# wujian16/Cornell-MOE

Measured on AMD Instinct MI355X. Metric: q-KG gradient evals/s (n=1000,d=8,q=4,10k MC), higher is better.
Workload: dtype f64

## Files before the change

### cornell_moe_amd/csrc/kg.hip

```cpp
#include "kg.hpp"

#include <algorithm>
#include <array>
#include <atomic>
#include <exception>
#include <mutex>
#include <thread>
#include <memory>
#include <optional>
#include <chrono>
#include <cmath>
#include <cstdlib>

#include "device_cov.hpp"
#include "fastmath.hpp"
#include "gemm128.hpp"
#include "kg_mc.hpp"
#include "kg_state.hpp"

namespace moe {

static thread_local int t_ens_members_hint = 1;
int ensemble_members_hint() { return t_ens_members_hint; }
void set_ensemble_members_hint(int members) { t_ens_members_hint = members > 1 ? members : 1; }
// ... 394 lines not shown
struct kg_dir_kernel_body {
  static __device__ __forceinline__ void run(const VIdx blockIdx, const VIdx gridDim, const void*, const KgTailParams& P, double* __restrict__ part, int slices) {
    __shared__ double red[4];
    const int k = blockIdx.x, e = blockIdx.y, sl = blockIdx.z;
    const int per = (P.num_local + slices - 1) / slices;
    const int i_lo = sl * per, i_hi = min(P.num_local, i_lo + per);
    const int m = P.m, g1 = 1 + P.g, d = P.cp.dim;
    const double* Xu = P.blob + (long)e * P.rec.stride + P.rec.XuP + (long)k * DP;
    DerivList none;
    none.g = 0;
    double xk[DP];
  #pragma unroll
    for (int kk = 0; kk < DP; ++kk) xk[kk] = Xu[kk];
    for (int b = 0; b < g1; ++b) {
      double acc[DP];
  #pragma unroll
      for (int dd = 0; dd < DP; ++dd) acc[dd] = 0.0;
      for (int i = i_lo + threadIdx.x; i < i_hi; i += 256) {
        const long w = (long)e * P.num_local + i;
        const double* xs = P.best_point + w * DP;
        double diff[DP];
        double r2 = 0.0;
  #pragma unroll
        for (int kk = 0; kk < DP; ++kk) {
          diff[kk] = xk[kk] - xs[kk];
          r2 = fma(diff[kk] * diff[kk], P.cp.inv_l2[kk], r2);
        }
        const Radial rd = radial_scalars(P.cp.type, P.cp.alpha, r2);
        const double bt = P.beta[w * m + k * g1 + b];
  #pragma unroll
        for (int dd = 0; dd < DP; ++dd)
          if (dd < d) acc[dd] = fma(bt, grad_cov_entry<DP>(P.cp, rd, diff, b, 0, dd, P.derivs, none), acc[dd]);
      }
  #pragma unroll
      for (int dd = 0; dd < DP; ++dd) {
        if (dd < d) {
          const double tot = block_sum_256(acc[dd], red);
          if (threadIdx.x == 0) part[((long)e * P.ngrad + (k * g1 + b) * d + dd) * slices + sl] = tot;
        }
      }
    }
  }
};
template <int DP>
__global__ __launch_bounds__(256) void kg_dir_kernel(KgTailParams P, double* __restrict__ part, int slices) {
  kg_dir_kernel_body<DP>::run(MOE_VBLOCK, MOE_VGRID, nullptr, P, part, slices);
}

inline int dir_slices(int num_local) { return std::max(1, std::min(kDirSlices, (num_local + 255) / 256)); }
inline double* dir_partials(const KgTailParams& P) {
  return P.TBpart + (long)P.E * (P.chunks + 1) * (long)P.m * P.N;
}

template <int DP>
void launch_dir(const KgTailParams& P, hipStream_t s) {
  const int slices = dir_slices(P.num_local);
  launch_kernel_ens<kg_dir_kernel_body<DP>, 256>(kg_dir_kernel<DP>, dim3(P.q, P.E, slices), dim3(256), 0, s, P, dir_partials(P), slices);
}

template <int DP, int MU>
void launch_sw_inst(const KgTailParams& P, hipStream_t s) {
  dim3 grid((P.num_local + P.sw_chunk - 1) / P.sw_chunk, P.E);
  const size_t shm = (P.SW == nullptr) ? sizeof(double) * (size_t)P.N * P.m : 0;
  auto kern = kg_sw_kernel<DP, MU>;
  if (shm > 48 * 1024)
    MOE_HIP_CHECK(hipFuncSetAttribute(reinterpret_cast<const void*>(kern), hipFuncAttributeMaxDynamicSharedMemorySize, (int)shm));
  launch_kernel_ens<kg_sw_kernel_body<DP, MU>, 256>(kern, grid, dim3(256), shm, s, P);
}

template <int DP>
void launch_sw_dp(const KgTailParams& P, hipStream_t s) {
  if (P.m <= 4)
    launch_sw_inst<DP, 4>(P, s);
  else if (P.m <= 8)
    launch_sw_inst<DP, 8>(P, s);
  else if (P.m <= 16)
    launch_sw_inst<DP, 16>(P, s);
  else if (P.m <= 32)
    launch_sw_inst<DP, 32>(P, s);
  else if (P.m <= 64)
    launch_sw_inst<DP, 64>(P, s);
  else {
    if (P.SW == nullptr) throw Error(MOE_ERR_RUNTIME, "m > 64 needs the precomputed W^T T");
    dim3 grid((P.num_local + P.sw_chunk - 1) / P.sw_chunk, P.E);
    launch_kernel_ens<kg_sw_kernel_body<DP, 1, 2>, 256>(kg_sw_kernel<DP, 1, 2>, grid, dim3(256), 0, s, P);
  }
  launch_dir<DP>(P, s);
}

void launch_tail(const KgTailParams& P, hipStream_t s) {
  switch (P.cp.dp) {
    case 4: launch_sw_dp<4>(P, s); break;
    case 8: launch_sw_dp<8>(P, s); break;
    case 12: launch_sw_dp<12>(P, s); break;
    case 16: launch_sw_dp<16>(P, s); break;
    case 24: launch_sw_dp<24>(P, s); break;
    case 32: launch_sw_dp<32>(P, s); break;
    default: throw Error(MOE_ERR_RUNTIME, "unsupported padded dimension");
  }
  dim3 gtb((P.N + 255) / 256, P.chunks, P.E);
  if (P.m <= 4)
    launch_kernel_ens<kg_tb_kernel_body<4>, 256>(kg_tb_kernel<4>, gtb, dim3(256), 0, s, P, 0);
  else if (P.m <= 8)
    launch_kernel_ens<kg_tb_kernel_body<8>, 256>(kg_tb_kernel<8>, gtb, dim3(256), 0, s, P, 0);
  else if (P.m <= 16)
    launch_kernel_ens<kg_tb_kernel_body<16>, 256>(kg_tb_kernel<16>, gtb, dim3(256), 0, s, P, 0);
// ... 73 lines not shown
__global__ __launch_bounds__(256) void kg_fused_sample_kernel(KgTailParams P, const double* __restrict__ X, int n,
                                                             double* __restrict__ SWpart) {
  kg_fused_sample_kernel_body<DP, MU, COV>::run(MOE_VBLOCK, MOE_VGRID, nullptr, P, X, n, SWpart);
}

template <int DP, int MU, int COV>
struct kg_fused_c_kernel_body {
  static __device__ __forceinline__ void run(const VIdx blockIdx, const VIdx gridDim, const void*, const KgTailParams& P, const double* __restrict__ SWpart, int slices) {
    __shared__ double etab[kExpTabLen];
    const int e = blockIdx.y, m = P.m;
    const int i = blockIdx.x * 256 + threadIdx.x;
    if (threadIdx.x < kExpTabLen) etab[threadIdx.x] = kExp2Tab64[threadIdx.x];
    __syncthreads();
    if (i >= P.num_local) return;
    const long w = (long)e * P.num_local + i;
    double xs[DP], sw[MU], cv[MU];
  #pragma unroll
    for (int k = 0; k < DP; ++k) xs[k] = P.best_point[w * DP + k] * P.cp.inv_l[k];
  #pragma unroll
    for (int c = 0; c < MU; ++c) {
      sw[c] = 0.0;
      for (int sl = 0; sl < slices; ++sl) sw[c] += SWpart[(w * slices + sl) * MU + c];
    }
    const double* rec = P.blob + (long)e * P.rec.stride;
    const double* Lsm = rec + P.rec.L;
  #pragma unroll
    for (int r = 0; r < MU; ++r) {
      cv[r] = 0.0;
      if (r < m) {
        const double* Xu = rec + P.rec.XuP + (long)r * DP;
        double r2 = 1.0e-300;
  #pragma unroll
        for (int k = 0; k < DP; ++k) {
          const double dlt = Xu[k] * P.cp.inv_l[k] - xs[k];
          r2 = fma(dlt, dlt, r2);
        }
        double R = P.cp.alpha * (radial_base<COV>(r2, etab) - sw[r]);
  #pragma unroll
        for (int c = 0; c < MU; ++c)
          if (c < r) R -= Lsm[r + c * m] * cv[c];
        cv[r] = R / Lsm[r + r * m];
        P.C[w * m + r] = cv[r];
      }
    }
  }
};
template <int DP, int MU, int COV>
__global__ __launch_bounds__(256) void kg_fused_c_kernel(KgTailParams P, const double* __restrict__ SWpart, int slices) {
  kg_fused_c_kernel_body<DP, MU, COV>::run(MOE_VBLOCK, MOE_VGRID, nullptr, P, SWpart, slices);
}

template <int DP, int MU, int COV>
struct kg_fused_point_kernel_body {
  static __device__ __forceinline__ void run(const VIdx blockIdx, const VIdx gridDim, const void*, const KgTailParams& P, const double* __restrict__ X, int n) {
    __shared__ double etab[kExpTabLen];
    __shared__ double St[kFusedTile][DP];
    __shared__ double Bt[kFusedTile][MU];
    const int row = blockIdx.x * 256 + threadIdx.x;
    const int chunk = blockIdx.y, e = blockIdx.z;
    const int m = P.m;
    const int i0 = chunk * P.chunk_len, cnt = min(P.num_local - i0, P.chunk_len);
    if (threadIdx.x < kExpTabLen) etab[threadIdx.x] = kExp2Tab64[threadIdx.x];
    for (int t = threadIdx.x; t < kFusedTile * DP; t += 256) {
      const int ii = t / DP, k = t % DP;
      St[ii][k] = (ii < cnt) ? P.best_point[((long)e * P.num_local + i0 + ii) * DP + k] * P.cp.inv_l[k] : 0.0;
    }
    for (int t = threadIdx.x; t < kFusedTile * MU; t += 256) {
      const int ii = t / MU, c = t % MU;
      Bt[ii][c] = (ii < cnt && c < m) ? P.beta[((long)e * P.num_local + i0 + ii) * m + c] : 0.0;
    }
    __syncthreads();
    const bool ok = row < n;
    double xr[DP], acc[MU];
  #pragma unroll
    for (int k = 0; k < DP; ++k) xr[k] = ok ? X[(long)row * DP + k] * P.cp.inv_l[k] : 0.0;
  #pragma unroll
    for (int c = 0; c < MU; ++c) acc[c] = 0.0;
  #pragma unroll 2
    for (int ii = 0; ii < cnt; ++ii) {
      double r2 = 1.0e-300;
  #pragma unroll
      for (int k = 0; k < DP; ++k) {
        const double dlt = xr[k] - St[ii][k];
        r2 = fma(dlt, dlt, r2);
      }
      const double t = radial_base<COV>(r2, etab);
  #pragma unroll
      for (int c = 0; c < MU; ++c) acc[c] = fma(t, Bt[ii][c], acc[c]);
    }
    if (ok) {
      double* dst = P.TBpart + ((long)e * P.chunks + chunk) * m * P.N;
  #pragma unroll
      for (int c = 0; c < MU; ++c)
        if (c < m) dst[(long)c * P.N + row] = P.cp.alpha * acc[c];
    }
  }
};
template <int DP, int MU, int COV>
__global__ __launch_bounds__(256) void kg_fused_point_kernel(KgTailParams P, const double* __restrict__ X, int n) {
  kg_fused_point_kernel_body<DP, MU, COV>::run(MOE_VBLOCK, MOE_VGRID, nullptr, P, X, n);
}

template <int DP, int MU, int COV>
struct kg_fused_pair_kernel_body {
  static constexpr int SB = kFusedChunk / 8;
  static constexpr int SROW = DP + 2;
  static constexpr int NW = 8, PB = 4;
  static __device__ __forceinline__ void run(const VIdx blockIdx, const VIdx gridDim, const void*, const KgTailParams& P, const double* __restrict__ X, int n, double* __restrict__ SWpart) {
    static_assert(MU <= 4 && kFusedChunk == 128, "4 point blocks x MU sums per lane");
    __shared__ double etab[kExpTabLen];
    __shared__ __attribute__((aligned(16))) double St[kFusedChunk][SROW];
    __shared__ __attribute__((aligned(16))) double Bt[kFusedChunk][MU];
    __shared__ __attribute__((aligned(16))) double Xt[256][SROW];
    __shared__ __attribute__((aligned(16))) double Wt[256][MU];
    __shared__ double Sx[NW][kFusedChunk][MU];
    const int lane = threadIdx.x & 63, wave = threadIdx.x >> 6;
    const int a = lane >> 3, b = lane & 7;
    const int chunk = blockIdx.y, e = blockIdx.z, m = P.m, N = P.N;
    const int i0 = chunk * P.chunk_len, cnt = min(P.num_local - i0, P.chunk_len);
    const long w0 = (long)e * P.num_local + i0;
    const int row0 = blockIdx.x * 256;
    if (threadIdx.x < kExpTabLen) etab[threadIdx.x] = kExp2Tab64[threadIdx.x];
    for (int t = threadIdx.x; t < kFusedChunk * DP; t += 64 * NW) {
      const int ii = t / DP, k = t % DP;
      St[ii][k] = (ii < cnt) ? P.best_point[(w0 + ii) * DP + k] * P.cp.inv_l[k] : 0.0;
    }
    for (int t = threadIdx.x; t < kFusedChunk * MU; t += 64 * NW) {
      const int ii = t / MU, c = t % MU;
      Bt[ii][c] = (ii < cnt && c < m) ? P.beta[(w0 + ii) * m + c] : 0.0;
    }
    for (int t = threadIdx.x; t < 256 * DP; t += 64 * NW) {
      const int jj = t / DP, k = t % DP;
      Xt[jj][k] = (row0 + jj < n) ? X[(long)(row0 + jj) * DP + k] * P.cp.inv_l[k] : 0.0;
    }
    {
      const double* We = P.W + (long)e * P.w_stride;
      for (int t = threadIdx.x; t < 256 * MU; t += 64 * NW) {
        const int jj = t % 256, c = t / 256;
        Wt[jj][c] = (row0 + jj < n && c < m) ? We[(long)c * N + row0 + jj] : 0.0;
      }
    }
    __syncthreads();
    double tb[PB][MU];
  #pragma unroll
    for (int pi = 0; pi < PB; ++pi)
  #pragma unroll
      for (int c = 0; c < MU; ++c) tb[pi][c] = 0.0;
    const int jw = wave * (8 * PB) + a;
  #pragma unroll 1
    for (int si = 0; si < SB; ++si) {
      const int ii = si * 8 + b;
      int hold = 0;
      asm volatile("" : "+v"(hold));
      double xs[DP], bs[MU], sw[MU];
  #pragma unroll
      for (int k = 0; k < DP; ++k) xs[k] = St[ii][k];
  #pragma unroll
      for (int c = 0; c < MU; ++c) {
        bs[c] = Bt[ii][c];
        sw[c] = 0.0;
      }
  #pragma unroll
      for (int pi = 0; pi < PB; ++pi) {
        const int jj = jw + pi * 8 + hold;
        double r2 = 1.0e-300;
  #pragma unroll
        for (int k = 0; k < DP; ++k) {
          const double dlt = Xt[jj][k] - xs[k];
          r2 = fma(dlt, dlt, r2);
        }
        const double t = radial_base<COV>(r2, etab);
  #pragma unroll
        for (int c = 0; c < MU; ++c) {
          tb[pi][c] = fma(t, bs[c], tb[pi][c]);
          sw[c] = fma(Wt[jj][c], t, sw[c]);
        }
      }
  #pragma unroll
      for (int c = 0; c < MU; ++c) {
        double v = sw[c];
        v += __shfl_xor(v, 8, 64);
        v += __shfl_xor(v, 16, 64);
        v += __shfl_xor(v, 32, 64);
        if (a == 0) Sx[wave][ii][c] = v;
      }
    }
    double* dst = P.TBpart + ((long)e * P.chunks + chunk) * m * N;
  #pragma unroll
    for (int pi = 0; pi < PB; ++pi)
  #pragma unroll
      for (int c = 0; c < MU; ++c) {
        double v = tb[pi][c];
        v += __shfl_xor(v, 1, 64);
        v += __shfl_xor(v, 2, 64);
        v += __shfl_xor(v, 4, 64);
        const int row = row0 + jw + pi * 8;
        if (b == 0 && c < m && row < n) dst[(long)c * N + row] = P.cp.alpha * v;
      }
    __syncthreads();
    const int slices = gridDim.x;
    for (int t = threadIdx.x; t < kFusedChunk * MU; t += 64 * NW) {
      const int ii = t / MU, c = t % MU;
      if (ii < cnt) {
        double v = Sx[0][ii][c];
  #pragma unroll
        for (int wv = 1; wv < NW; ++wv) v += Sx[wv][ii][c];
        SWpart[((w0 + ii) * slices + blockIdx.x) * MU + c] = v;
      }
    }
  }
};
template <int DP, int MU, int COV>
__global__ __launch_bounds__(512, 2) void kg_fused_pair_kernel(KgTailParams P, const double* __restrict__ X, int n, double* __restrict__ SWpart) {
  kg_fused_pair_kernel_body<DP, MU, COV>::run(MOE_VBLOCK, MOE_VGRID, nullptr, P, X, n, SWpart);
}

inline bool fused_tail_one_pass(int m, int dp) { return m <= 4 && dp <= 8 && env_int("MOE_KG_FUSED_ONE_PASS", 1) != 0; }

template <int DP, int MU, int COV>
void launch_fused_tail_cov(const KgTailParams& P, const double* X, int n, double* SWpart, int slices, hipStream_t s) {
  dim3 ga((P.num_local + 255) / 256, P.E, slices), gc((P.num_local + 255) / 256, P.E), gb((n + 255) / 256, P.chunks, P.E);
  if constexpr (MU <= 4 && DP <= 8) {
    if (fused_tail_one_pass(P.m, DP)) {
      launch_kernel_ens<kg_fused_pair_kernel_body<DP, MU, COV>, 512, 2>(kg_fused_pair_kernel<DP, MU, COV>, gb, dim3(512), 0, s, P, X, n, SWpart);
      launch_kernel_ens<kg_fused_c_kernel_body<DP, MU, COV>, 256>(kg_fused_c_kernel<DP, MU, COV>, gc, dim3(256), 0, s, P, SWpart, (int)gb.x);
      launch_dir<DP>(P, s);
      launch_gtb(P, s);
      MOE_HIP_CHECK(hipGetLastError());
      return;
    }
  }
  launch_kernel_ens<kg_fused_sample_kernel_body<DP, MU, COV>, 256>(kg_fused_sample_kernel<DP, MU, COV>, ga, dim3(256), 0, s, P, X, n, SWpart);
  launch_kernel_ens<kg_fused_c_kernel_body<DP, MU, COV>, 256>(kg_fused_c_kernel<DP, MU, COV>, gc, dim3(256), 0, s, P, SWpart, slices);
  launch_dir<DP>(P, s);
  launch_kernel_ens<kg_fused_point_kernel_body<DP, MU, COV>, 256>(kg_fused_point_kernel<DP, MU, COV>, gb, dim3(256), 0, s, P, X, n);
  launch_gtb(P, s);
  MOE_HIP_CHECK(hipGetLastError());
}

template <int DP, int MU>
void launch_fused_tail_inst(const KgTailParams& P, const double* X, int n, double* SWpart, int slices, hipStream_t s) {
  if (P.cp.type == MOE_COV_SQUARE_EXPONENTIAL)
    launch_fused_tail_cov<DP, MU, MOE_COV_SQUARE_EXPONENTIAL>(P, X, n, SWpart, slices, s);
  else
    launch_fused_tail_cov<DP, MU, MOE_COV_MATERN_NU_2P5>(P, X, n, SWpart, slices, s);
}

int fused_tail_slices(int , int num_local, int n, int num_cu, int m, int dp) {
  if (fused_tail_one_pass(m, dp)) return (n + 255) / 256;
  const long waves = (long)((num_local + 255) / 256) * 4;
  const long want = (long)num_cu * 4 * 4;
  int s = (int)std::min<long>(8, std::max<long>(1, (want + waves - 1) / waves));
  return std::max(1, std::min(s, (n + 63) / 64));
}

void launch_fused_tail(const KgTailParams& P, const double* X, int n, double* SWpart, int slices, hipStream_t s) {
  static_assert(kFusedChunk <= kFusedTile, "a chunk of samples is staged in one LDS tile");
  const bool m4 = P.m <= 4;
  switch (P.cp.dp) {
    case 4: m4 ? launch_fused_tail_inst<4, 4>(P, X, n, SWpart, slices, s) : launch_fused_tail_inst<4, 8>(P, X, n, SWpart, slices, s); break;
    case 8: m4 ? launch_fused_tail_inst<8, 4>(P, X, n, SWpart, slices, s) : launch_fused_tail_inst<8, 8>(P, X, n, SWpart, slices, s); break;
    case 12: m4 ? launch_fused_tail_inst<12, 4>(P, X, n, SWpart, slices, s) : launch_fused_tail_inst<12, 8>(P, X, n, SWpart, slices, s); break;
    case 16: m4 ? launch_fused_tail_inst<16, 4>(P, X, n, SWpart, slices, s) : launch_fused_tail_inst<16, 8>(P, X, n, SWpart, slices, s); break;
    case 24: m4 ? launch_fused_tail_inst<24, 4>(P, X, n, SWpart, slices, s) : launch_fused_tail_inst<24, 8>(P, X, n, SWpart, slices, s); break;
    case 32: m4 ? launch_fused_tail_inst<32, 4>(P, X, n, SWpart, slices, s) : launch_fused_tail_inst<32, 8>(P, X, n, SWpart, slices, s); break;
    default: throw Error(MOE_ERR_RUNTIME, "unsupported padded dimension");
  }
}

struct kg_sum_kernel_body {
  static __device__ __forceinline__ void run(const VIdx blockIdx, const VIdx gridDim, const void*, const KgTailParams& P, double* __restrict__ fin, const unsigned long long* __restrict__ counters, const int* __restrict__ flags) {
    __shared__ double red[4];
    const int e = blockIdx.x;
    const double bp = P.blob[(long)e * P.rec.stride + P.rec_bp];
    double acc = 0.0;
    for (int i = threadIdx.x; i < P.num_local; i += 256) acc += bp + P.best_value[(long)e * P.num_local + i];
    const double tot = block_sum_256(acc, red);
    if (threadIdx.x == 0) {
      fin[4 * e] = tot;
      fin[4 * e + 1] = (double)counters[2 * e];
      fin[4 * e + 2] = (double)counters[2 * e + 1];
      fin[4 * e + 3] = (double)flags[e];
    }
  }
};
__global__ __launch_bounds__(256) void kg_sum_kernel(KgTailParams P, double* __restrict__ fin, const unsigned long long* __restrict__ counters,
                                                     const int* __restrict__ flags) {
  kg_sum_kernel_body::run(MOE_VBLOCK, MOE_VGRID, nullptr, P, fin, counters, flags);
}

struct EventTimer {
  hipEvent_t a = nullptr, b = nullptr;
  bool on = false;
  EventTimer() = default;
  EventTimer(const EventTimer&) = delete;
  EventTimer& operator=(const EventTimer&) = delete;
  ~EventTimer() {
    if (a != nullptr) (void)hipEventDestroy(a);
    if (b != nullptr) (void)hipEventDestroy(b);
  }
  void start(hipStream_t s) {
    on = Recorder::current() == nullptr;
// ... 825 lines not shown
    launch_mc(mp, dp, pl.G, pl.xlds, pl.blocks, pl.waves, pl.shm, s);
  else if (pl.variant == 2)
    launch_mc_stream(mp, dp, pl.G, pl.blocks, pl.waves, pl.shm, s);
  else
    launch_mc_block(mp, dp, pl.G, pl.tr, pl.num_lds_tiles, pl.blocks, pl.waves, s);
  t_mc.stop(s);
  return mp;
}

KgTailParams launch_tail_step(GpDev& gp, const KgDims& k, const McPlan& pl, const KgMcParams& mp, const KgRecords& R,
                              double* dBlobP, const double* dNormalsP, const BatchLayout& bl, double* dFin, int out_stride,
                              EventTimer& t_cov, EventTimer& t_tail, hipStream_t s) {
  const int E = k.E, N = k.N, n = k.n, m = k.m, num_local = k.num_local;
  KgTailParams tl;
  tl.cp = gp.cp;
  tl.derivs = gp.derivs;
  tl.u = k.u;
  tl.q = k.q;
  tl.m = m;
  tl.g = k.g;
  tl.N = N;
  tl.E = E;
  tl.num_local = num_local;
  tl.first_sample = k.first_sample;
  tl.ngrad = k.ngrad;
  tl.chunks = (num_local + pl.chunk_len - 1) / pl.chunk_len;
  tl.chunk_len = pl.chunk_len;
  tl.sw_chunk = ((long)E * num_local / kSwChunk >= 1024) ? kSwChunk : 16;
  tl.T = gp.kT.p;
  tl.SW = nullptr;
  tl.W = mp.W;
  tl.w_stride = mp.w_stride;
  tl.Gm = gp.dE.p + bl.col_grad0(0) * N;
  tl.g_stride = (long)k.ngrad * N;
  tl.Linv = gp.dLinv.p;
  tl.ldL = gp.ldL;
  tl.tri_work = gp.dEK.p;
  tl.work = gp.dVE.p;
  tl.blob = dBlobP;
  tl.rec = R.rec;
  tl.rec_bp = R.rec_bp;
  tl.best_point = gp.kBestPoint.p;
  tl.best_value = gp.kBestValue.p;
  tl.beta = gp.kBeta.p;
  tl.normals = dNormalsP;
  tl.C = gp.kC.p;
  tl.TBpart = gp.kTB.p;
  tl.out = gp.kOut.p;
  tl.out_stride = out_stride;
  if (pl.fused_tail) {
    t_cov.start(s);
    t_cov.stop(s);
    t_tail.start(s);
    const int slices = fused_tail_slices(E, num_local, n, gp.num_cu, m, k.dp);
    gp.kSW.reserve((size_t)E * num_local * slices * 8);
    launch_fused_tail(tl, gp.dX.p, n, gp.kSW.p, slices, s);
    gp.kZcPart.reserve((size_t)E * ((num_local + zc_chunk_len(m) - 1) / zc_chunk_len(m)) * m * m);
    launch_zc(tl, gp.kZcPart.p, s, !zc_sum_in_finish(m, num_local));
  } else if (k.want_grad) {
    DerivList none;
    none.g = 0;
    for (int i = 0; i < kMaxDerivs; ++i) none.idx[i] = 0;
    t_cov.start(s);
    launch_cov_build(gp.cp, gp.dX.p, n, gp.derivs, gp.kBestPoint.p, E * num_local, none, nullptr, gp.kT.p, N, 0, s, true);
    t_cov.stop(s);
    t_tail.start(s);
    if (m > 8 || (size_t)N * m * sizeof(double) > 96 * 1024) {
      gp.kSW.reserve((size_t)m * E * num_local);
      const int sw_slices = N >= 1024 ? 8 : (N >= 256 ? 4 : 1);
      if (sw_slices > 1) gp.kSWpart.reserve((size_t)sw_slices * m * num_local * E);
      if (m > 64 && sw_slices > 1) {
        MOE_HIP_CHECK(hipFuncSetAttribute(reinterpret_cast<const void*>(kg_sw128_kernel), hipFuncAttributeMaxDynamicSharedMemorySize,
                                          (int)g128::kSmemBytes));
        double* sw_part_p = gp.kSWpart.p;
        launch_kernel_ens<kg_sw128_kernel_body, 256, 2>(kg_sw128_kernel, dim3((num_local + g128::TM - 1) / g128::TM, sw_slices, E), dim3(256), g128::kSmemBytes, s, tl,
                   sw_part_p, sw_slices);
        launch_sum_slices(gp.kSWpart.p, sw_slices, (long)m * num_local * E, gp.kSW.p, s);
      } else {
        launch_gemm_tn_splitk(m, num_local, N, tl.W, N, gp.kT.p, N, gp.kSW.p, gp.kSWpart.p, sw_slices, s, E, tl.w_stride, (long)num_local * N);
      }
      tl.SW = gp.kSW.p;
    }
    launch_tail(tl, s);
    gp.kZcPart.reserve((size_t)E * ((num_local + zc_chunk_len(m) - 1) / zc_chunk_len(m)) * m * m);
    launch_zc(tl, gp.kZcPart.p, s, !zc_sum_in_finish(m, num_local));
  } else {
    const unsigned long long* ctr_p = gp.kCounters.p;
    const int* flags_p = gp.kStateI.p;
    launch_kernel_ens<kg_sum_kernel_body, 256>(kg_sum_kernel, dim3(E), dim3(256), 0, s, tl, dFin, ctr_p, flags_p);
  }
  MOE_HIP_CHECK(hipGetLastError());
  return tl;
}

void launch_grad_finish(GpDev& gp, const KgDims& k, const KgStateParams& sp, const KgTailParams& tl, const KgRecords& R, double* dBlobP,
                        double* dFin, int out_stride, hipStream_t s) {
  const int m = k.m, num_local = k.num_local;
  KgFinishParams fp;
  fp.E = k.E;
  fp.q = k.q;
  fp.m = m;
  fp.g = k.g;
  fp.d = k.d;
  fp.ng = k.ngrad;
  fp.num_mc = k.num_mc;
  fp.first_sample = k.first_sample;
  fp.blob = dBlobP;
  fp.rec_stride = R.rec.stride;
  fp.rec_L = R.rec.L;
  fp.out = gp.kOut.p;
  fp.out_stride = out_stride;
  fp.winner = sp.winner;
  fp.gmu = sp.gmu;
  fp.dL = sp.dL;
  fp.fin = dFin;
  fp.counters = gp.kCounters.p;
  fp.flags = gp.kStateI.p;
  fp.dir_part = dir_partials(tl);
  fp.dir_slices = dir_slices(num_local);
  fp.zc_part = zc_sum_in_finish(m, num_local) ? gp.kZcPart.p : nullptr;
  fp.zc_chunks = (num_local + zc_chunk_len(m) - 1) / zc_chunk_len(m);
  fp.zc_gs = zc_sum_lanes(m);
  fp.best_value = gp.kBestValue.p;
  fp.num_local = num_local;
  fp.rec_bp = R.rec_bp;
  launch_kg_finish(fp, dFin + (size_t)k.E * (1 + k.qd + 3), s);
}

KgPending enqueue_results(GpDev& gp, const KgDims& k, const double* dFin, size_t n_ctr, bool want_best_points,
                          std::shared_ptr<std::array<EventTimer, 4>> timers, std::chrono::steady_clock::time_point wall0, hipStream_t s) {
  const int E = k.E, m = k.m, d = k.d, dp = k.dp, num_local = k.num_local, qd = k.qd;
  const bool want_grad = k.want_grad;
  const int fin_stride = (want_grad ? 1 + qd : 1) + 3;
  const size_t n_out = (size_t)fin_stride * E;
  gp.hKgOut.reserve(n_out);
  double* out = gp.hKgOut.p;
  copy_async(out, dFin, sizeof(double) * n_out, hipMemcpyDeviceToHost, s, true);
#if MOE_BLOCK_PROF
  auto prof_p = std::make_shared<std::vector<unsigned long long>>(16);
  copy_async(prof_p->data(), gp.kCounters.p + n_ctr - 16, sizeof(unsigned long long) * 16, hipMemcpyDeviceToHost, s);
#endif
  const bool fetch_bp = want_best_points && E == 1;
  auto bp_p = std::make_shared<std::vector<double>>();
  if (fetch_bp) {
    bp_p->resize((size_t)num_local * dp);
    gp.kBestPoint.download(bp_p->data(), bp_p->size(), s);
  }
  GpDev* gpp = &gp;
  KgPending pending;
  pending.collect = [=](double* kg_sum, double* grad_sum, double* best_points, moe_kg_stats_t* stats) {
    GpDev& gp = *gpp;
    gp.use_device();
    if (stats) std::memset(stats, 0, sizeof(*stats));
    MOE_HIP_CHECK(hipStreamSynchronize(s));
#if MOE_BLOCK_PROF
    {
      const unsigned long long* w = prof_p->data();
      const double tot = (double)(w[0] + w[1] + w[2] + w[3]);
      if (tot > 0 && w[8] > 0)
        std::fprintf(stderr,
                     "[moe prof] wave-0 cycles: ticket %.1f%%  z/beta/scan %.1f%%  weights %.1f%%  line search %.1f%%;  inside "
                     "%llu passes: accumulate %.0f  reduce %.0f  barrier %.0f  post %.0f  (cycles per pass; line search total "
                     "%.0f per pass)\n",
                     100.0 * w[0] / tot, 100.0 * w[1] / tot, 100.0 * w[2] / tot, 100.0 * w[3] / tot, w[8],
                     (double)w[4] / w[8], (double)w[5] / w[8], (double)w[6] / w[8], (double)w[7] / w[8], (double)w[3] / w[8]);
      if (w[10] > 0)
        std::fprintf(stderr, "[moe prof] gradient passes: %llu, %.0f cycles each (all phases); cycles per SAMPLE: total %.0f, in passes %.0f\n",
                     w[10], (double)w[9] / w[10], tot / (w[10] / 6.0), (double)(w[4] + w[5] + w[6] + w[7]) / (w[10] / 6.0));
      if (w[10] > 0)
        std::fprintf(stderr, "[moe prof] per sample: z/beta %.0f, scan %.0f cycles\n", (double)w[11] / (w[10] / 6.0), (double)w[12] / (w[10] / 6.0));
      if (w[10] > 0 && w[8] > 0)
        std::fprintf(stderr, "[moe prof] outside the passes, cycles per pass: gradient post + trial-line set-up %.0f, Armijo dispatch / decisions %.0f, "
                     "LimitUpdate + re-evaluation set-up + step end %.0f\n", (double)w[13] / w[8], (double)w[14] / w[8], (double)w[15] / w[8]);
// ... 55 lines not shown
  const int d = k.d, dp = k.dp, u = k.u, m = k.m, A = k.A, E = k.E, size = k.size, N = k.N, qd = k.qd;
  const McPlan pl = plan_mc(gp, k, bounds, Xq_all, Xp, weight_table_gb);

  const auto wall0 = std::chrono::steady_clock::now();

  std::vector<double> U_all((size_t)E * u * d), extra_all((size_t)E * A * d), disc_all((size_t)E * A * size);
  for (int e = 0; e < E; ++e) {
    double* U = &U_all[(size_t)e * u * d];
    const double* Xq = Xq_all + (size_t)e * q * d;
    std::copy(Xq, Xq + (size_t)q * d, U);
    if (p > 0) std::copy(Xp, Xp + (size_t)p * d, U + (size_t)q * d);
    double* ds = &disc_all[(size_t)e * A * size];
    for (int i = 0; i < u; ++i) {
      const double* src = (disc_head != nullptr && i < q) ? disc_head + (size_t)i * d : U + (size_t)i * d;
      std::copy(src, src + size, ds + (size_t)i * size);
    }
    std::copy(discrete, discrete + (size_t)P * size, ds + (size_t)u * size);
    double* ex = &extra_all[(size_t)e * A * d];
    for (int j = 0; j < A; ++j) {
      for (int kk = 0; kk < size; ++kk) ex[(size_t)j * d + kk] = ds[(size_t)j * size + kk];
      for (int kk = size; kk < d; ++kk) ex[(size_t)j * d + kk] = 1.0;
    }
  }
  const TabParams tp = table_rows(gp, k, pl.G, Xq_all, Xp, disc_head);
  const KgRecords R = fill_records(gp, k, pl, tp, bounds, U_all, disc_all);
  const double* blob = gp.hKgIn.p;
  const size_t blob_size = R.blob_size;
  const long num_norm = (long)((num_mc + 1) / 2) * m;

  auto timers = std::make_shared<std::array<EventTimer, 4>>();
  EventTimer &t_mc = (*timers)[0], &t_cov = (*timers)[1], &t_tail = (*timers)[2], &t_state = (*timers)[3];
  t_state.start(s);
  StateAppendix apx;
  apx.doubles = blob_size + (size_t)num_norm;
  apx.fill = [&](double* dst) {
    std::memcpy(dst, blob, sizeof(double) * blob_size);
    std::memcpy(dst + blob_size, normals, sizeof(double) * num_norm);
  };
  const KgStateEnqueued se = enqueue_kg_state_batch(gp, U_all.data(), u, want_grad ? q : 0, extra_all.data(), A, E, &apx);
  double* dBlobP = const_cast<double*>(gp.dAppendix);
  const double* dNormalsP = gp.dAppendix + blob_size;
  const KgStateParams sp = launch_state_algebra(gp, k, se, R, dBlobP, best_so_far, s);
  double* dFin = gp.kStateD.p + (size_t)E * qd * (1 + (want_grad ? m * (m + 1) / 2 : 0));

  const long tab_stride = (long)pl.ntiles * dp * 64;
  gp.kTab.reserve((size_t)tab_stride * E + (size_t)dp * 64);
  gp.kBestPoint.reserve((size_t)E * num_local * dp);
  gp.kBestValue.reserve((size_t)E * num_local);
  gp.kBeta.reserve((size_t)E * num_local * m + 64);
  const size_t n_ctr = (size_t)2 * E + (size_t)E * (kTicketStride / 2) + 32;
  gp.kCounters.reserve(n_ctr);
  const int out_stride = 1 + m * m + 2 * k.ngrad;
  gp.kOut.reserve((size_t)out_stride * E);
  if (want_grad) {
    const int chunks = (num_local + pl.chunk_len - 1) / pl.chunk_len;
    if (!pl.fused_tail) gp.kT.reserve((size_t)N * E * num_local);
    gp.kC.reserve((size_t)E * num_local * m);
    gp.kTB.reserve((size_t)E * (chunks + 1) * m * N + (size_t)E * k.ngrad * kDirSlices);
  }

  {
    dim3 grid((unsigned)((tab_stride + 255) / 256), E);
    const double *dXp = gp.dX.p, *dUnionP = gp.dUnion;
    double* dTabP = gp.kTab.p;
    unsigned long long* dCtrP = gp.kCounters.p;
    launch_kernel_ens<build_xs_tab_kernel_body, 256>(build_xs_tab_kernel, grid, dim3(256), 0, s, dXp, k.n, dUnionP, u, dp, pl.ntiles, tp, dTabP, tab_stride,
                                                     pl.pair_rows, dCtrP, (long)n_ctr);
    MOE_HIP_CHECK(hipGetLastError());
  }

  const KgMcParams mp = launch_mc_step(gp, k, pl, gd, tp, R, dBlobP, dNormalsP, se.bl, tab_stride, n_ctr, t_state, t_mc, s);
  {
    const int info[8] = {pl.variant,
                         ((pl.variant == 0 && pl.xlds) ? 1 : 0) | (pl.far_frame ? 2 : 0) | (pl.wide_frame ? 4 : 0) | (pl.lane_kernel ? 8 : 0) |
                             (pl.start_table ? 16 : 0),
                         pl.waves, pl.variant == 1 ? pl.tr : pl.wide_lds_tiles, pl.weight_table ? 1 : 0, pl.fused_tail ? 1 : 0, pl.blocks,
                         pl.prep ? 1 : 0};
    std::copy(info, info + 8, gp.last_info);
  }

  const KgTailParams tl = launch_tail_step(gp, k, pl, mp, R, dBlobP, dNormalsP, se.bl, dFin, out_stride, t_cov, t_tail, s);
  if (want_grad) {
    launch_grad_finish(gp, k, sp, tl, R, dBlobP, dFin, out_stride, s);
    t_tail.stop(s);
  }
  return enqueue_results(gp, k, dFin, n_ctr, want_best_points, timers, wall0, s);
}

int kg_max_batch(const GpDev& gp, int P, int q, int p, int num_local, bool want_grad, double budget_gb) {
  const double N = gp.N, g1 = 1 + gp.g, u = q + p, m = u * g1, A = u + P;
  const double ngrad = want_grad ? q * g1 * gp.d : 0.0;
  const bool fused = fused_tail_taken(want_grad, gp.g, (int)m);
  const double chunks = std::ceil((double)num_local / tail_chunk_len(fused, (int)m));
  double doubles = N * (m + ngrad + A) + 3.0 * N * m + (double)num_local * (gp.dp + 1 + 2 * m) +
                   (want_grad ? (double)q * gp.d * m * (m + 1) / 2 : 0.0);
  if (want_grad) doubles += (fused ? 0.0 : N * (double)num_local) + (chunks + 1.0) * m * N;
  if (want_grad && !fused) doubles += 9.0 * m * (double)num_local;
  const double slots1 = gp.g <= 4 ? g1 : (gp.g <= 8 ? 9.0 : 13.0);
  doubles += (gp.n + u + 64.0) * slots1 * (double)num_local;
  doubles += 8.0 * N * m + (m * m + A * (1.0 + m + gp.d) + u * gp.dp + 8.0);
  const double per_eval_gb = 8.0 * doubles / 1e9;
  return (int)std::max(1.0, std::floor(budget_gb / std::max(per_eval_gb, 1e-9)));
}

void kg_evaluate_batch(GpDev& gp, int num_fidelity, const moe_gd_params_t& gd, const double* bounds, const double* discrete,
                       int P, const double* Xq_all, int num_evals, const double* Xp, int q, int p, int num_mc,
                       double best_so_far, const double* normals, int first_sample, int num_local, bool want_grad,
                       double* kg_sum, double* grad_sum, double* best_points, moe_kg_stats_t* stats, const double* disc_head) {
  const double budget = (double)env_int("MOE_KG_BATCH_GB", 48);
  const int max_e = kg_max_batch(gp, P, q, p, num_local, want_grad, budget);
  if (num_evals <= max_e) {
    KgPending pending = kg_launch(gp, num_fidelity, gd, bounds, discrete, P, Xq_all, num_evals, Xp, q, p, num_mc, best_so_far,
                                  normals, first_sample, num_local, want_grad, best_points != nullptr, budget, disc_head);
    pending.collect(kg_sum, grad_sum, best_points, stats);
    return;
  }
  const size_t qd = (size_t)q * gp.d;
  moe_kg_stats_t total{}, part{};
  for (int e0 = 0; e0 < num_evals; e0 += max_e) {
    const int ne = std::min(max_e, num_evals - e0);
    KgPending pending = kg_launch(gp, num_fidelity, gd, bounds, discrete, P, Xq_all + (size_t)e0 * qd, ne, Xp, q, p, num_mc,
                                  best_so_far, normals, first_sample, num_local, want_grad, false, budget, disc_head);
    pending.collect(kg_sum + e0, grad_sum ? grad_sum + (size_t)e0 * qd : nullptr, nullptr, stats ? &part : nullptr);
    total.posterior_mean_evals += part.posterior_mean_evals;
    total.posterior_grad_evals += part.posterior_grad_evals;
    total.ms_state += part.ms_state;
    total.ms_mc += part.ms_mc;
    total.ms_tail += part.ms_tail;
  }
  if (stats) *stats = total;
}

}
```

### cornell_moe_amd/csrc/kg_state.hip

```cpp
#include "kg_state.hpp"

#include <algorithm>

#include "device_cov.hpp"

namespace moe {

namespace {

constexpr size_t kLdsBudget = 150 * 1024;

__device__ __forceinline__ double wave_sum64(double v) {
#pragma unroll
  for (int off = 32; off > 0; off >>= 1) v += __shfl_xor(v, off, 64);
  return v;
}

__device__ __forceinline__ double pts_cov(const CovParams& cp, const double* p1, const double* p2, int d, int a, int b,
                                          const DerivList& d1, const DerivList& d2) {
  const PointDiff df{p1, p2};
  const Radial rd = pair_radial(cp, df, d);
  return cov_entry_g(cp, rd, df, a, b, d1, d2);
}

// ... 232 lines not shown
  const double mine = (lane < P.dir_slices) ? p[lane] : 0.0;
  double tot = 0.0;
  for (int sl = 0; sl < P.dir_slices; ++sl) tot += __shfl(mine, sl, 64);
  return tot;
}

__device__ __forceinline__ void finish_component(const KgFinishParams& P, int e, int idx, int lane, double zmc, double kg_sum) {
  const int m = P.m, g1 = 1 + P.g, d = P.d, qd = P.q * P.d;
  const double* GTB = P.out + (long)e * P.out_stride + 1 + m * m + P.ng;
  const int k = idx / d, dd = idx - k * d;
  double direct = 0.0;
  for (int b = 0; b < g1; ++b) {
    const int gc = (k * g1 + b) * d + dd;
    const double dir = dir_sum(P, e, gc, lane);
    direct += dir - GTB[gc];
  }
  if (lane != 0) return;
  double val = -(direct - zmc);
  if (P.winner[e] == k && P.first_sample == 0) val += (double)P.num_mc * P.gmu[(long)e * qd + idx];
  double* fin = P.fin + (long)e * (1 + qd + 3);
  fin[1 + idx] = val;
  if (idx == 0) {
    fin[0] = kg_sum;
    fin[1 + qd] = (double)P.counters[2 * e];
    fin[2 + qd] = (double)P.counters[2 * e + 1];
    fin[3 + qd] = (double)P.flags[e];
  }
}

struct kg_finish_kernel_body {
  static __device__ __forceinline__ void run(const VIdx blockIdx, const VIdx gridDim, const void*, const KgFinishParams& P, const double* __restrict__ Y) {
    const int idx = blockIdx.x, e = blockIdx.y, lane = threadIdx.x;
    const int m = P.m, qd = P.q * P.d;
    const int tri = m * (m + 1) / 2;
    const double* dl = P.dL + ((long)e * qd + idx) * tri;
    const double* y = Y + (long)e * tri;
    double acc = 0.0;
  #pragma unroll 4
    for (int t = lane; t < tri; t += 64) acc = fma(y[t], dl[t], acc);
    const double zmc = wave_sum64(acc);
    finish_component(P, e, idx, lane, zmc, P.out[(long)e * P.out_stride]);
  }
};
__global__ __launch_bounds__(64) void kg_finish_kernel(KgFinishParams P, const double* __restrict__ Y) {
  kg_finish_kernel_body::run(MOE_VBLOCK, MOE_VGRID, nullptr, P, Y);
}

struct kg_finish_small_kernel_body {
  static __device__ __forceinline__ void run(const VIdx blockIdx, const VIdx gridDim, const void*, const KgFinishParams& P) {
    __shared__ double zcs[64], Lp[36], Yp[36], red[4];
    const int idx = blockIdx.x, e = blockIdx.y, tid = threadIdx.x;
    const int m = P.m, qd = P.q * P.d;
    const int tri = m * (m + 1) / 2;
    {
      const int gs = P.zc_gs, per_block = 256 / gs;
      for (int base = 0; base < m * m; base += per_block) {
        const int oo = base + tid / gs, g = tid % gs;
        const bool ok = oo < m * m;
        const double* p = P.zc_part + (long)e * P.zc_chunks * m * m + (ok ? oo : 0);
        double v = 0.0;
  #pragma unroll 8
        for (int ch = g; ch < P.zc_chunks; ch += gs) v += p[(long)ch * m * m];
        for (int off = gs >> 1; off > 0; off >>= 1) v += __shfl_xor(v, off, 64);
        if (ok && g == 0) zcs[oo] = v;
      }
    }
    double kg_sum = 0.0;
    if (idx == 0) {
      const double bp = P.blob[(long)e * P.rec_stride + P.rec_bp];
      double acc = 0.0;
  #pragma unroll 8
      for (int i = tid; i < P.num_local; i += 256) acc += bp + P.best_value[(long)e * P.num_local + i];
      const double w = wave_sum64(acc);
      __syncthreads();
      if ((tid & 63) == 0) red[tid >> 6] = w;
      __syncthreads();
      kg_sum = (red[0] + red[1]) + (red[2] + red[3]);
    }
    __syncthreads();
    const double* Lg = P.blob + (long)e * P.rec_stride + P.rec_L;
    if (tid < m * m) {
      const int l = tid % m, j = tid / m;
      if (l >= j) {
        Lp[l * (l + 1) / 2 + j] = Lg[tid];
        Yp[l * (l + 1) / 2 + j] = zcs[tid];
      }
    }
    __syncthreads();
    for (int rr = m - 1; rr >= 0; --rr) {
      if (tid <= rr) {
        double t = Yp[rr * (rr + 1) / 2 + tid];
  #pragma unroll 4
        for (int i = m - 1; i > rr; --i) t = fma(-Lp[i * (i + 1) / 2 + rr], Yp[i * (i + 1) / 2 + tid], t);
        Yp[rr * (rr + 1) / 2 + tid] = t / Lp[rr * (rr + 1) / 2 + rr];
      }
    }
    __syncthreads();
    if (tid >= 64) return;
    const int lane = tid;
    const double* dl = P.dL + ((long)e * qd + idx) * tri;
    double acc = 0.0;
  #pragma unroll 4
    for (int t = lane; t < tri; t += 64) acc = fma(Yp[t], dl[t], acc);
    const double zmc = wave_sum64(acc);
    finish_component(P, e, idx, lane, zmc, kg_sum);
  }
};
__global__ __launch_bounds__(256) void kg_finish_small_kernel(KgFinishParams P) {
  kg_finish_small_kernel_body::run(MOE_VBLOCK, MOE_VGRID, nullptr, P);
}

template <class K>
void opt_in_lds(K kern, size_t shm) {
  if (shm > 48 * 1024)
    MOE_HIP_CHECK(hipFuncSetAttribute(reinterpret_cast<const void*>(kern), hipFuncAttributeMaxDynamicSharedMemorySize, (int)shm));
}

}

void launch_kg_state(const KgStateParams& P, hipStream_t s) {
  const size_t mm = (size_t)P.m * P.m;
  const size_t room = kLdsBudget / sizeof(double) - mm;
  const int rchunk = (int)std::max<size_t>(1, std::min<size_t>((size_t)std::max(P.A, 1), room / P.m));
  const size_t shm = sizeof(double) * (mm + (size_t)rchunk * P.m);
  opt_in_lds(kg_state_kernel, shm);
  launch_kernel_ens<kg_state_kernel_body, 256>(kg_state_kernel, dim3(P.E), dim3(256), shm, s, P, rchunk);
  MOE_HIP_CHECK(hipGetLastError());
}

void launch_kg_dchol(const KgStateParams& P, hipStream_t s) {
  if (P.ng <= 0) return;
  const size_t shm = sizeof(double) * ((size_t)P.m * (P.m + 1) / 2 + 3 * (size_t)P.m);
  opt_in_lds(kg_dchol_kernel, shm);
  launch_kernel_ens<kg_dchol_kernel_body, 256>(kg_dchol_kernel, dim3(P.q * P.d, P.E), dim3(256), shm, s, P);
  MOE_HIP_CHECK(hipGetLastError());
}

void launch_kg_finish(const KgFinishParams& P, double* Y, hipStream_t s) {
  if (P.zc_part != nullptr) {
    launch_kernel_ens<kg_finish_small_kernel_body, 256>(kg_finish_small_kernel, dim3(P.q * P.d, P.E), dim3(256), 0, s, P);
  } else {
    const size_t shm = sizeof(double) * (size_t)P.m * (P.m + 1);
    opt_in_lds(kg_y_kernel, shm);
    launch_kernel_ens<kg_y_kernel_body, 128>(kg_y_kernel, dim3(P.E), dim3(128), shm, s, P, Y);
    launch_kernel_ens<kg_finish_kernel_body, 64>(kg_finish_kernel, dim3(P.q * P.d, P.E), dim3(64), 0, s, P, (const double*)Y);
  }
  MOE_HIP_CHECK(hipGetLastError());
}

}
```

### cornell_moe_amd/csrc/kg_state.hpp

```cpp
#pragma once
#include "gp.hpp"

namespace moe {

struct KgStateParams {
  CovParams cp;
  DerivList derivs;
  double noise[kMaxDerivs + 1];
  double mean;
  double best_so_far;
  int E, u, q, m, g, d, dp, A, ng;
  const double* gkk;
  const double* gx;
  int gkk_slices, gx_slices;
  const double* ek;
  const double* U;
  const double* extra;
  double* blob;
  int rec_stride, rec_L, rec_mu_disc, rec_C_disc, rec_bp;
  int* flags;
  int* winner;
  double* gmu;
  double* dL;
};

void launch_kg_state(const KgStateParams& P, hipStream_t s);
void launch_kg_dchol(const KgStateParams& P, hipStream_t s);

struct KgFinishParams {
  int E, q, m, g, d, ng, num_mc, first_sample;
  const double* blob;
  int rec_stride, rec_L;
  const double* out;
  int out_stride;
  const int* winner;
  const double* gmu;
  const double* dL;
  double* fin;
  const unsigned long long* counters;
  const int* flags;
  const double* dir_part;
  int dir_slices;
  const double* zc_part;
  int zc_chunks, zc_gs;
  const double* best_value;
  int num_local, rec_bp;
};
void launch_kg_finish(const KgFinishParams& P, double* Y, hipStream_t s);

}
```

Baseline: 1944.

## Compute Zc directly from TB sums, dropping the per-sample SW pass

The default fused tail no longer runs the pair kernel, the C-solve kernel or the separate Zc partial reduction. The point kernel now also evaluates the m extra rows for the Xu points to get K(Xu,best) partials. A new single-block-per-ensemble kernel reduces TB against W over N, combines that with the K-block partials, and triangular-solves to write Zc straight into the output. The finish kernel reads Zc from there. This removes the per-sample SW work and the C buffer, at the cost of a serial-per-ensemble reduction over N in one block.

```diff
diff --git a/cornell_moe_amd/csrc/kg.hip b/cornell_moe_amd/csrc/kg.hip
--- a/cornell_moe_amd/csrc/kg.hip
+++ b/cornell_moe_amd/csrc/kg.hip
@@ -470,6 +470,10 @@
   return P.TBpart + (long)P.E * (P.chunks + 1) * (long)P.m * P.N;
 }
 
+__host__ __device__ inline double* kb_partials(const KgTailParams& P) {
+  return P.TBpart + (long)P.E * (P.chunks + 1) * (long)P.m * P.N + (long)P.E * P.ngrad * kDirSlices;
+}
+
 template <int DP>
 void launch_dir(const KgTailParams& P, hipStream_t s) {
   const int slices = dir_slices(P.num_local);
@@ -649,7 +653,7 @@
 
 template <int DP, int MU, int COV>
 struct kg_fused_point_kernel_body {
-  static __device__ __forceinline__ void run(const VIdx blockIdx, const VIdx gridDim, const void*, const KgTailParams& P, const double* __restrict__ X, int n) {
+  static __device__ __forceinline__ void run(const VIdx blockIdx, const VIdx gridDim, const void*, const KgTailParams& P, const double* __restrict__ X, int n, int kb_rows) {
     __shared__ double etab[kExpTabLen];
     __shared__ double St[kFusedTile][DP];
     __shared__ double Bt[kFusedTile][MU];
@@ -667,10 +671,12 @@
       Bt[ii][c] = (ii < cnt && c < m) ? P.beta[((long)e * P.num_local + i0 + ii) * m + c] : 0.0;
     }
     __syncthreads();
+    if (row >= n + kb_rows) return;
     const bool ok = row < n;
+    const double* __restrict__ xp = ok ? X + (long)row * DP : P.blob + (long)e * P.rec.stride + P.rec.XuP + (long)(row - n) * DP;
     double xr[DP], acc[MU];
   #pragma unroll
-    for (int k = 0; k < DP; ++k) xr[k] = ok ? X[(long)row * DP + k] * P.cp.inv_l[k] : 0.0;
+    for (int k = 0; k < DP; ++k) xr[k] = xp[k] * P.cp.inv_l[k];
   #pragma unroll
     for (int c = 0; c < MU; ++c) acc[c] = 0.0;
   #pragma unroll 2
@@ -690,147 +696,123 @@
   #pragma unroll
       for (int c = 0; c < MU; ++c)
         if (c < m) dst[(long)c * P.N + row] = P.cp.alpha * acc[c];
+    } else {
+      double* dst = kb_partials(P) + ((long)e * P.chunks + chunk) * m * m;
+  #pragma unroll
+      for (int c = 0; c < MU; ++c)
+        if (c < m) dst[c * m + (row - n)] = P.cp.alpha * acc[c];
     }
   }
 };
 template <int DP, int MU, int COV>
-__global__ __launch_bounds__(256) void kg_fused_point_kernel(KgTailParams P, const double* __restrict__ X, int n) {
-  kg_fused_point_kernel_body<DP, MU, COV>::run(MOE_VBLOCK, MOE_VGRID, nullptr, P, X, n);
-}
-
-template <int DP, int MU, int COV>
-struct kg_fused_pair_kernel_body {
-  static constexpr int SB = kFusedChunk / 8;
-  static constexpr int SROW = DP + 2;
-  static constexpr int NW = 8, PB = 4;
-  static __device__ __forceinline__ void run(const VIdx blockIdx, const VIdx gridDim, const void*, const KgTailParams& P, const double* __restrict__ X, int n, double* __restrict__ SWpart) {
-    static_assert(MU <= 4 && kFusedChunk == 128, "4 point blocks x MU sums per lane");
-    __shared__ double etab[kExpTabLen];
-    __shared__ __attribute__((aligned(16))) double St[kFusedChunk][SROW];
-    __shared__ __attribute__((aligned(16))) double Bt[kFusedChunk][MU];
-    __shared__ __attribute__((aligned(16))) double Xt[256][SROW];
-    __shared__ __attribute__((aligned(16))) double Wt[256][MU];
-    __shared__ double Sx[NW][kFusedChunk][MU];
-    const int lane = threadIdx.x & 63, wave = threadIdx.x >> 6;
-    const int a = lane >> 3, b = lane & 7;
-    const int chunk = blockIdx.y, e = blockIdx.z, m = P.m, N = P.N;
-    const int i0 = chunk * P.chunk_len, cnt = min(P.num_local - i0, P.chunk_len);
-    const long w0 = (long)e * P.num_local + i0;
-    const int row0 = blockIdx.x * 256;
-    if (threadIdx.x < kExpTabLen) etab[threadIdx.x] = kExp2Tab64[threadIdx.x];
-    for (int t = threadIdx.x; t < kFusedChunk * DP; t += 64 * NW) {
-      const int ii = t / DP, k = t % DP;
-      St[ii][k] = (ii < cnt) ? P.best_point[(w0 + ii) * DP + k] * P.cp.inv_l[k] : 0.0;
-    }
-    for (int t = threadIdx.x; t < kFusedChunk * MU; t += 64 * NW) {
-      const int ii = t / MU, c = t % MU;
-      Bt[ii][c] = (ii < cnt && c < m) ? P.beta[(w0 + ii) * m + c] : 0.0;
-    }
-    for (int t = threadIdx.x; t < 256 * DP; t += 64 * NW) {
-      const int jj = t / DP, k = t % DP;
-      Xt[jj][k] = (row0 + jj < n) ? X[(long)(row0 + jj) * DP + k] * P.cp.inv_l[k] : 0.0;
-    }
+__global__ __launch_bounds__(256) void kg_fused_point_kernel(KgTailParams P, const double* __restrict__ X, int n, int kb_rows) {
+  kg_fused_point_kernel_body<DP, MU, COV>::run(MOE_VBLOCK, MOE_VGRID, nullptr, P, X, n, kb_rows);
+}
+
+template <int MU>
+struct kg_zc_direct_kernel_body {
+  static __device__ __forceinline__ void run(const VIdx blockIdx, const VIdx gridDim, const void*, const KgTailParams& P, const double* __restrict__ TBsum) {
+    __shared__ double red[4][MU * MU], kbs[256], Bs[MU * MU], As[MU * MU];
+    const int e = blockIdx.x, tid = threadIdx.x, lane = tid & 63, wave = tid >> 6;
+    const int m = P.m, N = P.N, mm = m * m;
+    const double* __restrict__ tb = TBsum + (long)e * m * N;
+    const double* __restrict__ We = P.W + (long)e * P.w_stride;
+    double acc[MU][MU];
+  #pragma unroll
+    for (int c = 0; c < MU; ++c)
+  #pragma unroll
+      for (int r = 0; r < MU; ++r) acc[c][r] = 0.0;
+  #pragma unroll 2
+    for (int row = tid; row < N; row += 256) {
+      double t[MU], w[MU];
+  #pragma unroll
+      for (int c = 0; c < MU; ++c) {
+        t[c] = (c < m) ? tb[(long)c * N + row] : 0.0;
+        w[c] = (c < m) ? We[(long)c * N + row] : 0.0;
+      }
+  #pragma unroll
+      for (int c = 0; c < MU; ++c)
+  #pragma unroll
+        for (int r = 0; r < MU; ++r) acc[c][r] = fma(t[c], w[r], acc[c][r]);
+    }
+  #pragma unroll
+    for (int c = 0; c < MU; ++c)
+  #pragma unroll
+      for (int r = 0; r < MU; ++r) {
+        const double v = wave_sum64(acc[c][r]);
+        if (lane == 0) red[wave][c * MU + r] = v;
+      }
     {
-      const double* We = P.W + (long)e * P.w_stride;
-      for (int t = threadIdx.x; t < 256 * MU; t += 64 * NW) {
-        const int jj = t % 256, c = t / 256;
-        Wt[jj][c] = (row0 + jj < n && c < m) ? We[(long)c * N + row0 + jj] : 0.0;
+      const int groups = 256 / mm;
+      const int o = tid % mm, g = tid / mm;
+      const double* __restrict__ kp = kb_partials(P) + (long)e * P.chunks * mm + o;
+      double v = 0.0;
+      if (g < groups) {
+  #pragma unroll 4
+        for (int ch = g; ch < P.chunks; ch += groups) v += kp[(long)ch * mm];
       }
+      kbs[tid] = v;
     }
     __syncthreads();
-    double tb[PB][MU];
-  #pragma unroll
-    for (int pi = 0; pi < PB; ++pi)
-  #pragma unroll
-      for (int c = 0; c < MU; ++c) tb[pi][c] = 0.0;
-    const int jw = wave * (8 * PB) + a;
-  #pragma unroll 1
-    for (int si = 0; si < SB; ++si) {
-      const int ii = si * 8 + b;
-      int hold = 0;
-      asm volatile("" : "+v"(hold));
-      double xs[DP], bs[MU], sw[MU];
-  #pragma unroll
-      for (int k = 0; k < DP; ++k) xs[k] = St[ii][k];
-  #pragma unroll
-      for (int c = 0; c < MU; ++c) {
-        bs[c] = Bt[ii][c];
-        sw[c] = 0.0;
-      }
-  #pragma unroll
-      for (int pi = 0; pi < PB; ++pi) {
-        const int jj = jw + pi * 8 + hold;
-        double r2 = 1.0e-300;
-  #pragma unroll
-        for (int k = 0; k < DP; ++k) {
-          const double dlt = Xt[jj][k] - xs[k];
-          r2 = fma(dlt, dlt, r2);
-        }
-        const double t = radial_base<COV>(r2, etab);
-  #pragma unroll
-        for (int c = 0; c < MU; ++c) {
-          tb[pi][c] = fma(t, bs[c], tb[pi][c]);
-          sw[c] = fma(Wt[jj][c], t, sw[c]);
+    if (tid < mm) {
+      const int groups = 256 / mm;
+      const int c = tid / m, r = tid - c * m;
+      double kb = 0.0;
+      for (int g = 0; g < groups; ++g) kb += kbs[g * mm + tid];
+      const int o = c * MU + r;
+      Bs[tid] = kb - ((red[0][o] + red[1][o]) + (red[2][o] + red[3][o]));
+    }
+    __syncthreads();
+    const double* Lsm = P.blob + (long)e * P.rec.stride + P.rec.L;
+    if (tid < mm) {
+      const int a = tid / m, r = tid - a * m;
+      double v = 0.0;
+      for (int c = a; c < m; ++c) v = fma(Lsm[c + a * m], Bs[c * m + r], v);
+      As[tid] = v;
+    }
+    __syncthreads();
+    if (tid < m) {
+      double* out = P.out + (long)e * P.out_stride + 1;
+      double zc[MU];
+  #pragma unroll
+      for (int j = 0; j < MU; ++j) {
+        zc[j] = 0.0;
+        if (j < m) {
+          double v = As[tid * m + j];
+  #pragma unroll
+          for (int k = 0; k < MU; ++k)
+            if (k < j) v = fma(-zc[k], Lsm[j + k * m], v);
+          zc[j] = v / Lsm[j + j * m];
+          out[tid + j * m] = zc[j];
         }
       }
-  #pragma unroll
-      for (int c = 0; c < MU; ++c) {
-        double v = sw[c];
-        v += __shfl_xor(v, 8, 64);
-        v += __shfl_xor(v, 16, 64);
-        v += __shfl_xor(v, 32, 64);
-        if (a == 0) Sx[wave][ii][c] = v;
-      }
-    }
-    double* dst = P.TBpart + ((long)e * P.chunks + chunk) * m * N;
-  #pragma unroll
-    for (int pi = 0; pi < PB; ++pi)
-  #pragma unroll
-      for (int c = 0; c < MU; ++c) {
-        double v = tb[pi][c];
-        v += __shfl_xor(v, 1, 64);
-        v += __shfl_xor(v, 2, 64);
-        v += __shfl_xor(v, 4, 64);
-        const int row = row0 + jw + pi * 8;
-        if (b == 0 && c < m && row < n) dst[(long)c * N + row] = P.cp.alpha * v;
-      }
-    __syncthreads();
-    const int slices = gridDim.x;
-    for (int t = threadIdx.x; t < kFusedChunk * MU; t += 64 * NW) {
-      const int ii = t / MU, c = t % MU;
-      if (ii < cnt) {
-        double v = Sx[0][ii][c];
-  #pragma unroll
-        for (int wv = 1; wv < NW; ++wv) v += Sx[wv][ii][c];
-        SWpart[((w0 + ii) * slices + blockIdx.x) * MU + c] = v;
-      }
-    }
-  }
-};
-template <int DP, int MU, int COV>
-__global__ __launch_bounds__(512, 2) void kg_fused_pair_kernel(KgTailParams P, const double* __restrict__ X, int n, double* __restrict__ SWpart) {
-  kg_fused_pair_kernel_body<DP, MU, COV>::run(MOE_VBLOCK, MOE_VGRID, nullptr, P, X, n, SWpart);
-}
-
-inline bool fused_tail_one_pass(int m, int dp) { return m <= 4 && dp <= 8 && env_int("MOE_KG_FUSED_ONE_PASS", 1) != 0; }
+    }
+  }
+};
+template <int MU>
+__global__ __launch_bounds__(256) void kg_zc_direct_kernel(KgTailParams P, const double* __restrict__ TBsum) {
+  kg_zc_direct_kernel_body<MU>::run(MOE_VBLOCK, MOE_VGRID, nullptr, P, TBsum);
+}
+
+inline bool fused_tail_sw_free() { return env_int("MOE_KG_FUSED_ONE_PASS", 1) != 0; }
 
 template <int DP, int MU, int COV>
 void launch_fused_tail_cov(const KgTailParams& P, const double* X, int n, double* SWpart, int slices, hipStream_t s) {
+  if (fused_tail_sw_free()) {
+    dim3 gb((n + P.m + 255) / 256, P.chunks, P.E);
+    launch_kernel_ens<kg_fused_point_kernel_body<DP, MU, COV>, 256>(kg_fused_point_kernel<DP, MU, COV>, gb, dim3(256), 0, s, P, X, n, P.m);
+    launch_dir<DP>(P, s);
+    launch_gtb(P, s);
+    const double* TBsum = P.TBpart + (long)P.E * P.chunks * (long)P.m * P.N;
+    launch_kernel_ens<kg_zc_direct_kernel_body<MU>, 256>(kg_zc_direct_kernel<MU>, dim3(P.E), dim3(256), 0, s, P, TBsum);
+    MOE_HIP_CHECK(hipGetLastError());
+    return;
+  }
   dim3 ga((P.num_local + 255) / 256, P.E, slices), gc((P.num_local + 255) / 256, P.E), gb((n + 255) / 256, P.chunks, P.E);
-  if constexpr (MU <= 4 && DP <= 8) {
-    if (fused_tail_one_pass(P.m, DP)) {
-      launch_kernel_ens<kg_fused_pair_kernel_body<DP, MU, COV>, 512, 2>(kg_fused_pair_kernel<DP, MU, COV>, gb, dim3(512), 0, s, P, X, n, SWpart);
-      launch_kernel_ens<kg_fused_c_kernel_body<DP, MU, COV>, 256>(kg_fused_c_kernel<DP, MU, COV>, gc, dim3(256), 0, s, P, SWpart, (int)gb.x);
-      launch_dir<DP>(P, s);
-      launch_gtb(P, s);
-      MOE_HIP_CHECK(hipGetLastError());
-      return;
-    }
-  }
   launch_kernel_ens<kg_fused_sample_kernel_body<DP, MU, COV>, 256>(kg_fused_sample_kernel<DP, MU, COV>, ga, dim3(256), 0, s, P, X, n, SWpart);
   launch_kernel_ens<kg_fused_c_kernel_body<DP, MU, COV>, 256>(kg_fused_c_kernel<DP, MU, COV>, gc, dim3(256), 0, s, P, SWpart, slices);
   launch_dir<DP>(P, s);
-  launch_kernel_ens<kg_fused_point_kernel_body<DP, MU, COV>, 256>(kg_fused_point_kernel<DP, MU, COV>, gb, dim3(256), 0, s, P, X, n);
+  launch_kernel_ens<kg_fused_point_kernel_body<DP, MU, COV>, 256>(kg_fused_point_kernel<DP, MU, COV>, gb, dim3(256), 0, s, P, X, n, 0);
   launch_gtb(P, s);
   MOE_HIP_CHECK(hipGetLastError());
 }
@@ -843,8 +825,7 @@
     launch_fused_tail_cov<DP, MU, MOE_COV_MATERN_NU_2P5>(P, X, n, SWpart, slices, s);
 }
 
-int fused_tail_slices(int , int num_local, int n, int num_cu, int m, int dp) {
-  if (fused_tail_one_pass(m, dp)) return (n + 255) / 256;
+int fused_tail_slices(int , int num_local, int n, int num_cu) {
   const long waves = (long)((num_local + 255) / 256) * 4;
   const long want = (long)num_cu * 4 * 4;
   int s = (int)std::min<long>(8, std::max<long>(1, (want + waves - 1) / waves));
@@ -1776,11 +1757,15 @@
     t_cov.start(s);
     t_cov.stop(s);
     t_tail.start(s);
-    const int slices = fused_tail_slices(E, num_local, n, gp.num_cu, m, k.dp);
-    gp.kSW.reserve((size_t)E * num_local * slices * 8);
-    launch_fused_tail(tl, gp.dX.p, n, gp.kSW.p, slices, s);
-    gp.kZcPart.reserve((size_t)E * ((num_local + zc_chunk_len(m) - 1) / zc_chunk_len(m)) * m * m);
-    launch_zc(tl, gp.kZcPart.p, s, !zc_sum_in_finish(m, num_local));
+    if (fused_tail_sw_free()) {
+      launch_fused_tail(tl, gp.dX.p, n, nullptr, 0, s);
+    } else {
+      const int slices = fused_tail_slices(E, num_local, n, gp.num_cu);
+      gp.kSW.reserve((size_t)E * num_local * slices * 8);
+      launch_fused_tail(tl, gp.dX.p, n, gp.kSW.p, slices, s);
+      gp.kZcPart.reserve((size_t)E * ((num_local + zc_chunk_len(m) - 1) / zc_chunk_len(m)) * m * m);
+      launch_zc(tl, gp.kZcPart.p, s, !zc_sum_in_finish(m, num_local));
+    }
   } else if (k.want_grad) {
     DerivList none;
     none.g = 0;
@@ -1818,7 +1803,7 @@
 }
 
 void launch_grad_finish(GpDev& gp, const KgDims& k, const KgStateParams& sp, const KgTailParams& tl, const KgRecords& R, double* dBlobP,
-                        double* dFin, int out_stride, hipStream_t s) {
+                        double* dFin, int out_stride, bool zc_direct, hipStream_t s) {
   const int m = k.m, num_local = k.num_local;
   KgFinishParams fp;
   fp.E = k.E;
@@ -1842,7 +1827,8 @@
   fp.flags = gp.kStateI.p;
   fp.dir_part = dir_partials(tl);
   fp.dir_slices = dir_slices(num_local);
-  fp.zc_part = zc_sum_in_finish(m, num_local) ? gp.kZcPart.p : nullptr;
+  fp.zc_part = (!zc_direct && zc_sum_in_finish(m, num_local)) ? gp.kZcPart.p : nullptr;
+  fp.zc_direct = zc_direct ? gp.kOut.p + 1 : nullptr;
   fp.zc_chunks = (num_local + zc_chunk_len(m) - 1) / zc_chunk_len(m);
   fp.zc_gs = zc_sum_lanes(m);
   fp.best_value = gp.kBestValue.p;
@@ -2004,11 +1990,12 @@
   gp.kCounters.reserve(n_ctr);
   const int out_stride = 1 + m * m + 2 * k.ngrad;
   gp.kOut.reserve((size_t)out_stride * E);
+  const bool sw_free = pl.fused_tail && fused_tail_sw_free();
   if (want_grad) {
     const int chunks = (num_local + pl.chunk_len - 1) / pl.chunk_len;
     if (!pl.fused_tail) gp.kT.reserve((size_t)N * E * num_local);
-    gp.kC.reserve((size_t)E * num_local * m);
-    gp.kTB.reserve((size_t)E * (chunks + 1) * m * N + (size_t)E * k.ngrad * kDirSlices);
+    if (!sw_free) gp.kC.reserve((size_t)E * num_local * m);
+    gp.kTB.reserve((size_t)E * (chunks + 1) * m * N + (size_t)E * k.ngrad * kDirSlices + (sw_free ? (size_t)E * chunks * m * m : 0));
   }
 
   {
@@ -2033,7 +2020,7 @@
 
   const KgTailParams tl = launch_tail_step(gp, k, pl, mp, R, dBlobP, dNormalsP, se.bl, dFin, out_stride, t_cov, t_tail, s);
   if (want_grad) {
-    launch_grad_finish(gp, k, sp, tl, R, dBlobP, dFin, out_stride, s);
+    launch_grad_finish(gp, k, sp, tl, R, dBlobP, dFin, out_stride, sw_free, s);
     t_tail.stop(s);
   }
   return enqueue_results(gp, k, dFin, n_ctr, want_best_points, timers, wall0, s);
diff --git a/cornell_moe_amd/csrc/kg_state.hip b/cornell_moe_amd/csrc/kg_state.hip
--- a/cornell_moe_amd/csrc/kg_state.hip
+++ b/cornell_moe_amd/csrc/kg_state.hip
@@ -308,7 +308,9 @@
     const int idx = blockIdx.x, e = blockIdx.y, tid = threadIdx.x;
     const int m = P.m, qd = P.q * P.d;
     const int tri = m * (m + 1) / 2;
-    {
+    if (P.zc_part == nullptr) {
+      if (tid < m * m) zcs[tid] = P.zc_direct[(long)e * P.out_stride + tid];
+    } else {
       const int gs = P.zc_gs, per_block = 256 / gs;
       for (int base = 0; base < m * m; base += per_block) {
         const int oo = base + tid / gs, g = tid % gs;
@@ -393,7 +395,7 @@
 }
 
 void launch_kg_finish(const KgFinishParams& P, double* Y, hipStream_t s) {
-  if (P.zc_part != nullptr) {
+  if (P.zc_part != nullptr || P.zc_direct != nullptr) {
     launch_kernel_ens<kg_finish_small_kernel_body, 256>(kg_finish_small_kernel, dim3(P.q * P.d, P.E), dim3(256), 0, s, P);
   } else {
     const size_t shm = sizeof(double) * (size_t)P.m * (P.m + 1);
diff --git a/cornell_moe_amd/csrc/kg_state.hpp b/cornell_moe_amd/csrc/kg_state.hpp
--- a/cornell_moe_amd/csrc/kg_state.hpp
+++ b/cornell_moe_amd/csrc/kg_state.hpp
@@ -43,6 +43,7 @@
   int dir_slices;
   const double* zc_part;
   int zc_chunks, zc_gs;
+  const double* zc_direct;
   const double* best_value;
   int num_local, rec_bp;
 };
```

Result: faster. 1991 (median of 6 runs) (+2.4%).
